# Mingqj/OcRFDet

Hardware: AMD Instinct MI355X
Metric: BEV voxels/sec + rendered views/sec, 6-cam 256x704 (higher is better)
Workload: dtype f32

## Files before the change

include/ocrf_hip.h:

```cpp
#ifndef OCRF_HIP_H
#define OCRF_HIP_H

#include <stddef.h>
#include <stdint.h>

#ifdef __cplusplus
extern "C" {
#endif

typedef void *ocrf_stream_t;

const char *ocrf_version(void);


void bev_pool_v2(int c, int n_intervals, const float *depth, const float *feat,
                 const int *ranks_depth, const int *ranks_feat, const int *ranks_bev,
                 const int *interval_starts, const int *interval_lengths, float *out);

void bev_pool_v2_grad(int c, int n_intervals, const float *out_grad, const float *depth,
                      const float *feat, const int *ranks_depth, const int *ranks_feat,
                      const int *ranks_bev, const int *interval_starts,
                      const int *interval_lengths, float *depth_grad, float *feat_grad);

int ocrf_bev_pool_v2(int c, int n_intervals, int n_points, long n_voxels, const float *depth, const float *feat,
// ... 166 lines not shown
                             float *heatmap, float *anno_box, long long *ind, unsigned char *mask, float *counts,
                             void *workspace, size_t workspace_bytes, ocrf_stream_t stream);
size_t ocrf_center_head_heatmap_loss_workspace_bytes(int B, int T, const int *ncls, int HW);
int ocrf_center_head_heatmap_loss(int B, int T, const int *ncls, int HW, const float *const *logits,
                                  const float *heatmap, const float *counts, float loss_weight, float *const *clipped,
                                  float *out, float *dens, void *workspace, size_t workspace_bytes,
                                  ocrf_stream_t stream);
int ocrf_center_head_heatmap_loss_backward(int B, int T, const int *ncls, int HW, const float *const *logits,
                                           const float *heatmap, const float *dens, const float *grad_out,
                                           float loss_weight, float *const *grad_logits, ocrf_stream_t stream);
size_t ocrf_center_head_reg_loss_workspace_bytes(int B, int T);
int ocrf_center_head_reg_loss(int B, int T, int HW, int max_objs, int with_velocity, const float *const *heads,
                              const float *anno_box, const long long *ind, const unsigned char *mask,
                              const float *code_weights, const float *counts, float loss_weight, float *out,
                              float *dens, void *workspace, size_t workspace_bytes, ocrf_stream_t stream);
int ocrf_center_head_reg_loss_backward(int B, int T, int HW, int max_objs, int with_velocity,
                                       const float *const *heads, const float *anno_box, const long long *ind,
                                       const unsigned char *mask, const float *code_weights, const float *dens,
                                       const float *grad_out, float loss_weight, float *const *grad_heads,
                                       ocrf_stream_t stream);

#define OCRF_CD_MAX_TASKS 8
#define OCRF_CD_MAX_CLASSES 8
#define OCRF_CD_MAX_NUM 1024
size_t ocrf_center_decode_workspace_bytes(int B, int T, int max_num, int post_max_size);
int ocrf_center_decode(int B, int T, const int *ncls, int H, int W, const float *const *heads, int with_velocity,
                       int norm_bbox, int max_num, int pre_max_size, int post_max_size, float out_size_factor,
                       const float *voxel_size, const float *pc_range, int has_coder_score_threshold,
                       float coder_score_threshold, const float *post_center_range, int has_score_threshold,
                       float score_threshold, const float *post_center_limit_range, const int *nms_circle,
                       const double *nms_threshold, const float *rescale_factor, float *boxes, float *scores,
                       int *labels, int *counts, void *workspace, size_t workspace_bytes, ocrf_stream_t stream);

int ocrf_lss_prepare(int B, int N, int D, int H, int W, const float *frustum, const float *cams,
                     const float *grid_lower_host, const float *grid_interval_host, int gx, int gy, int gz,
                     int *ranks_bev, int *ranks_depth, int *ranks_feat, int *interval_starts,
                     int *interval_lengths, int *counts, void *workspace, size_t workspace_bytes,
                     ocrf_stream_t stream);
size_t ocrf_lss_prepare_workspace_bytes(int B, int N, int D, int H, int W, int gx, int gy, int gz);
int ocrf_ht_prepare(int B, int N, int Z, int n_pillars, int Wf, int Hf, int D, const float *ref_points,
                    const float *cams, const float *pc_range_host, float w_in, float h_in, float depth0,
                    float depth1, int *ranks_bev, int *ranks_depth, int *ranks_feat, int *interval_starts,
                    int *interval_lengths, int *counts, void *workspace, size_t workspace_bytes,
                    ocrf_stream_t stream);
size_t ocrf_ht_prepare_workspace_bytes(int B, int n_pillars);

int ocrf_geometry_blocks(int B, int N, const float *rots, const float *trans, const float *intrins,
                         const float *post_rots, const float *post_trans, const float *bda, const float *c2w,
                         int H_in, int W_in, float znear, float zfar, float *lss_block, float *ht_block,
                         float *camera_rows, ocrf_stream_t stream);

int ocrf_hoa_channel_stats(const float *x, int B, int C, int Y, int X, float *stats,
                           ocrf_stream_t stream);
int ocrf_hoa_opacity_mask_gate(const float *x, const float *stats, const float *opacity_bev,
                               const float *conv_w, int k, int B, int C, int Y, int X, float *mask,
                               float *gated, ocrf_stream_t stream);

int ocrf_hoa_dw3x3(const float *x, const float *w, const float *bias, int B, int C, int Y, int X, float *y,
                   ocrf_stream_t stream);
int ocrf_hoa_dw3x3_wgrad_bands(int Y);
int ocrf_hoa_dw3x3_wgrad(const float *x, const float *dy, int B, int C, int Y, int X, float *partial,
                         ocrf_stream_t stream);

int ocrf_hoa_height_attention(const float *x, int B, int C, int hid, int Y, int X, const float *w1,
                              const float *w2, float *gate, float *gated, void *workspace,
                              size_t workspace_bytes, ocrf_stream_t stream);
size_t ocrf_hoa_height_attention_workspace_bytes(int B, int C);

int ocrf_hoa_unet_block(const float *src0, const float *gate0, int C0, int H0, int W0, int mode,
                        const float *up_w, const float *up_b, int Cup, const float *src1,
                        const float *gate1, int C1, const float *dw_w, const float *dw_b,
                        const float *pw_w, const float *pw_b, int Cout, const float *addend, float *out,
                        float *partial_max, int B, int H, int W, ocrf_stream_t stream);
int ocrf_hoa_unet_tiles(int H, int W);
int ocrf_hoa_v2b_weights_len(void);
size_t ocrf_hoa_v2b_workspace_bytes(int B, int H, int W);
int ocrf_hoa_v2b_forward(const float *x, const float *position, const float *weights, int B, int H, int W,
                         void *workspace, size_t workspace_bytes, float *out, ocrf_stream_t stream);
int ocrf_hoa_height_gate_from_tiles(int B, int C, int hid, int n_tiles, const float *partial_max,
                                    const float *w1, const float *w2, float *gate, ocrf_stream_t stream);
int ocrf_hoa_gated_conv1x1(const float *x, const float *gate, int B, int C, int H, int W, const float *w,
                           const float *bias, float *out, ocrf_stream_t stream);

int ocrf_hoa1_forward(const float *opacity, const float *alpha, const float *weights, int B, int Y, int X,
                      float offset_scale, float *att_workspace, float *out, ocrf_stream_t stream);
int ocrf_hoa1_weights_len(void);

int ocrf_ht_project(int B, int N, int Z, int n_pillars, const float *ref_points, const float *cams,
                    const float *pc_range, float w_in, float h_in, float depth0, float depth1,
                    float *pix, unsigned char *mask, float *voxel, ocrf_stream_t stream);


int ocrf_prefilter(const float *x, int BN, int D, int C, int HW, float depth_threshold,
                   float semantic_threshold, float *depth, float *filter_depth, float *semantic,
                   float *feat_channels_last, ocrf_stream_t stream);

int ocrf_pillar_sample_mean(const float *imgs, const float *pix, const unsigned char *mask, float *avg,
                            int B, int N, int C, int Hi, int Wi, int ZQ, ocrf_stream_t stream);

int ocrf_retain_valid_pixels(const float *imgs, const float *pix, const unsigned char *mask,
                             const int *cam_sel, float *out, int B, int N, int C, int H, int W, int ZQ,
                             ocrf_stream_t stream);

int ocrf_gauss_heads(const float *bev, const float *rgb_avg, const float *params, int B, int C, int Zh,
                     int YX, float *opacity, float *scales, float *rotations, float *color,
                     ocrf_stream_t stream);
// ... 146 lines not shown
```

ocrfdet_amd/csrc/hoa.hip:

```cpp
#include <hip/hip_runtime.h>

#include <algorithm>

#include "hoa_gate.h"
#include "launch.h"
#include "ocrf_hip.h"

namespace {

constexpr int kBlock = 256;
int g_mg_groups = 0, g_mg_threads = kBlock, g_stats_threads = kBlock;

__device__ __forceinline__ float sigmoidf_(float v) { return 1.0f / (1.0f + __expf(-v)); }

__global__ __launch_bounds__(kBlock) void hoa_channel_stats_kernel(const float* __restrict__ x, int C,
                                                                   long plane, float* __restrict__ stats) {
  OCRF_MAIN_CHAIN_PRIO();
  const long pix = (long)blockIdx.x * blockDim.x + threadIdx.x;
  const int b = blockIdx.y;
  if (pix >= plane) return;
  const float* p = x + (long)b * C * plane + pix;
  float sum = 0.f, mx = -INFINITY;
  int c = 0;
  for (; c + 16 <= C; c += 16) {
    float v[16];
#pragma unroll
    for (int u = 0; u < 16; ++u) v[u] = p[(long)(c + u) * plane];
#pragma unroll
    for (int u = 0; u < 16; ++u) {
      sum += v[u];
      mx = fmaxf(mx, v[u]);
    }
  }
  for (; c < C; ++c) {
    const float v = p[(long)c * plane];
    sum += v;
    mx = fmaxf(mx, v);
  }
  stats[((long)b * 2 + 0) * plane + pix] = sum / (float)C;
  stats[((long)b * 2 + 1) * plane + pix] = mx;
}

struct MaskGateD1 {
  const float* d1; const float* pm; const float* out_w; const float* out_b; const float* g_w1; const float* g_w2;
  float* opacity_out; int tiles;
};
template <int VEC, int KT, bool FAST = false, bool D1 = false>
__global__ __launch_bounds__(kBlock) void hoa_mask_gate_kernel(
    const float* __restrict__ x, const float* __restrict__ stats, const float* __restrict__ opacity_bev,
    const float* __restrict__ conv_w, int k_rt, int C, int Y, int X, int groups, int n_rows,
    float* __restrict__ mask, float* __restrict__ gated, MaskGateD1 dd) {
  OCRF_MAIN_CHAIN_PRIO();
  const int k = KT ? KT : k_rt;
  const int nt = (int)blockDim.x;
  extern __shared__ __attribute__((aligned(16))) float s_dyn[];
  const int r = k / 2, tw = FAST ? X + 8 : ((VEC == 4) ? ((X + k - 1 + 3) & ~3) : (X + k - 1));
  constexpr int PL = FAST ? 1 : 0;
  float* s_w = s_dyn;
  float* s_s = s_dyn + ((VEC == 4) ? ((2 * k * k + 3) & ~3) : 2 * k * k);
  const long plane = (long)Y * X;
  const int b = blockIdx.z / groups, g = blockIdx.z % groups;
  const long p0 = (long)blockIdx.x * nt * VEC;
  const int row0 = (int)(p0 / X) - r;
  for (int i = threadIdx.x; i < 2 * k * k; i += nt) s_w[i] = conv_w[i];
  const long pix_e = p0 + (long)threadIdx.x * VEC;
  const int cpg_e = (C + groups - 1) / groups;
  const int c0_e = g * cpg_e, c1_e = min(C, c0_e + cpg_e);
  float4 first[5];
  const bool pre = (VEC == 4) && gated && pix_e < plane && c0_e + 5 <= c1_e;
  if constexpr (VEC == 4) {
    if (pre) {
      const float* pe = x + (long)b * C * plane + pix_e;
#pragma unroll
      for (int u = 0; u < 5; ++u) first[u] = *reinterpret_cast<const float4*>(pe + (long)(c0_e + u) * plane);
    }
  }
  __shared__ __attribute__((aligned(16))) float s_red[16 * 4];
  __shared__ float s_g[4], s_ow[16];
  float4 d1v[D1 ? 4 : 1];
  float4 pmv[hoa_gate::kPmRounds];
  float owv = 0.f;
  if constexpr (D1) {
    const long pc = pix_e < plane ? pix_e : plane - VEC;
#pragma unroll
    for (int c = 0; c < 4; ++c) d1v[c] = *reinterpret_cast<const float4*>(dd.d1 + ((long)b * 4 + c) * plane + pc);
    hoa_gate::pm_issue<4>(dd.pm, b, dd.tiles, (int)threadIdx.x, pmv);
    const int t = (int)threadIdx.x & 15;
    const float* src = t < 4 ? dd.out_w + t : (t == 4 ? dd.out_b : (t < 9 ? dd.g_w1 + (t - 5) : dd.g_w2 + (min(t, 12) - 9)));
    owv = *src;
  }
  if constexpr (FAST) {
    const int n_items = 2 * n_rows * 64, x4 = X >> 2;
    float4* s_s4 = reinterpret_cast<float4*>(s_s);
// ... 260 lines not shown
        const int sx = xx + j - 1;
        if (sx < 0 || sx >= X) continue;
        acc[i * 3 + j] = fmaf(g, px[(long)sy * X + sx], acc[i * 3 + j]);
      }
    }
  }
#pragma unroll
  for (int t = 0; t < 10; ++t) {
    float v = acc[t];
    for (int off = 32; off > 0; off >>= 1) v += __shfl_down(v, off);
    if ((threadIdx.x & 63) == 0) s_acc[threadIdx.x >> 6][t] = v;
  }
  __syncthreads();
  if (threadIdx.x < 10) {
    float v = 0.f;
    for (int wv = 0; wv < kBlock / 64; ++wv) v += s_acc[wv][threadIdx.x];
    partial[((long)bc * gridDim.x + band) * 10 + threadIdx.x] = v;
  }
}

}

namespace ocrf {
void hoa_tune(int key, int value) {
  if (key == 20 && value >= 0) g_mg_groups = value;
  if (key == 21 && (value == 64 || value == 128 || value == 256)) g_mg_threads = value;
  if (key == 22 && (value == 64 || value == 128 || value == 256)) g_stats_threads = value;
}
}

extern "C" {

int ocrf_hoa_dw3x3(const float* x, const float* w, const float* bias, int B, int C, int Y, int X, float* y,
                   ocrf_stream_t stream_) {
  if (!x || !w || !y || B <= 0 || C <= 0 || Y <= 0 || X <= 0 || (long)B * C > 65535) return (int)hipErrorInvalidValue;
  ocrf::launch(OCRF_K_HOA_DW3X3, hoa_dw3x3_kernel, dim3((X + 63) / 64, (Y + 3) / 4, B * C), dim3(kBlock), 0,
               static_cast<hipStream_t>(stream_), x, w, bias, C, Y, X, y);
  return (int)hipGetLastError();
}

int ocrf_hoa_dw3x3_wgrad_bands(int Y) { return (Y + kDwBand - 1) / kDwBand; }

int ocrf_hoa_dw3x3_wgrad(const float* x, const float* dy, int B, int C, int Y, int X, float* partial,
                         ocrf_stream_t stream_) {
  if (!x || !dy || !partial || B <= 0 || C <= 0 || Y <= 0 || X <= 0 || (long)B * C > 65535)
    return (int)hipErrorInvalidValue;
  ocrf::launch(OCRF_K_HOA_DW3X3_WGRAD, hoa_dw3x3_wgrad_kernel, dim3(ocrf_hoa_dw3x3_wgrad_bands(Y), B * C),
               dim3(kBlock), 0, static_cast<hipStream_t>(stream_), x, dy, Y, X, partial);
  return (int)hipGetLastError();
}

int ocrf_hoa_channel_stats(const float* x, int B, int C, int Y, int X, float* stats, ocrf_stream_t stream_) {
  hipStream_t stream = static_cast<hipStream_t>(stream_);
  if (!x || !stats || B <= 0 || C <= 0 || Y <= 0 || X <= 0) return (int)hipErrorInvalidValue;
  const long plane = (long)Y * X;
  const int nt = g_stats_threads;
  ocrf::launch(OCRF_K_HOA_STATS, hoa_channel_stats_kernel, dim3((unsigned)((plane + nt - 1) / nt), B), dim3(nt), 0, stream,
               x, C, plane, stats);
  return (int)hipGetLastError();
}

int ocrf_hoa_opacity_mask_gate(const float* x, const float* stats, const float* opacity_bev,
                               const float* conv_w, int k, int B, int C, int Y, int X, float* mask,
                               float* gated, ocrf_stream_t stream_) {
  hipStream_t stream = static_cast<hipStream_t>(stream_);
  if (!x || !stats || !opacity_bev || !conv_w || !mask || k <= 0 || (k & 1) == 0 || k > 15 || B <= 0 ||
      C <= 0 || Y <= 0 || X <= 0)
    return (int)hipErrorInvalidValue;
  const long plane = (long)Y * X;
  const bool vec4 = (X % 4 == 0) && ((reinterpret_cast<uintptr_t>(x) | reinterpret_cast<uintptr_t>(gated)) & 15u) == 0 &&
                    (X + 6) * 14 * 2 * 4 <= 60 * 1024;
  const int threads = g_mg_threads;
  const int per_wg = threads * (vec4 ? 4 : 1);
  const int n_rows = (per_wg + X - 2) / X + 1 + (k - 1);
  const bool fast = vec4 && k == 7 && X <= 256 && (reinterpret_cast<uintptr_t>(stats) & 15u) == 0;
  const int tw = fast ? X + 8 : (vec4 ? ((X + k - 1 + 3) & ~3) : (X + k - 1));
  const size_t lds = (size_t)((vec4 ? ((2 * k * k + 3) & ~3) : 2 * k * k) + 2 * n_rows * tw) * sizeof(float);
  if (lds > 64 * 1024) return (int)hipErrorInvalidValue;
  int groups = gated ? ((C >= 40) ? 4 : (C >= 16 ? 2 : 1)) : 1;
  if (gated && g_mg_groups > 0) groups = std::min(g_mg_groups, C);
  const dim3 grid((unsigned)((plane + per_wg - 1) / per_wg), 1, (unsigned)(B * groups));
#define OCRF_MASK_GATE(V, K, F)                                                                                       \
  ocrf::launch(OCRF_K_HOA_MASK_GATE, hoa_mask_gate_kernel<V, K, F, false>, grid, dim3(threads), lds, stream, x, stats, opacity_bev, \
               conv_w, k, C, Y, X, groups, n_rows, mask, gated, MaskGateD1{})
  if (fast) OCRF_MASK_GATE(4, 7, true);
  else if (vec4 && k == 7) OCRF_MASK_GATE(4, 7, false);
  else if (vec4) OCRF_MASK_GATE(4, 0, false);
  else if (k == 7) OCRF_MASK_GATE(1, 7, false);
  else OCRF_MASK_GATE(1, 0, false);
#undef OCRF_MASK_GATE
  return (int)hipGetLastError();
}


size_t ocrf_hoa_height_attention_workspace_bytes(int B, int C) {
  return (size_t)B * C * 64 * sizeof(float);
}

int ocrf_hoa_height_attention(const float* x, int B, int C, int hid, int Y, int X, const float* w1,
                              const float* w2, float* gate, float* gated, void* workspace,
                              size_t workspace_bytes, ocrf_stream_t stream_) {
  hipStream_t stream = static_cast<hipStream_t>(stream_);
  if (!x || !w1 || !w2 || !gate || B <= 0 || C <= 0 || (C % 4) != 0 || C > 64 || hid <= 0 || 4 * hid > 64 ||
      Y <= 0 || X <= 0 || !workspace || workspace_bytes < ocrf_hoa_height_attention_workspace_bytes(B, C))
    return (int)hipErrorInvalidValue;
  const long plane = (long)Y * X;
  int n_split = (int)((plane + 4095) / 4096);
  if (n_split > 64) n_split = 64;
  float* partial = static_cast<float*>(workspace);
  ocrf::launch(OCRF_K_HOA_HEIGHT_MAX, hoa_height_max_kernel, dim3(n_split, B * C), dim3(kBlock), 0, stream, x,
               plane, n_split, partial);
// ... 774 lines not shown
```

ocrfdet_amd/csrc/step.hip:

```cpp
#include <hip/hip_runtime.h>

#include <cstdint>
#include <cstring>
#include <tuple>
#include <type_traits>
#include <utility>
#include <vector>

#include "ocrf_hip.h"

namespace {

constexpr int kMaxArgs = 40;
constexpr int kMaxStreams = 8;

template <typename T>
T word_as(uint64_t w) {
  if constexpr (std::is_pointer_v<T>) {
    return reinterpret_cast<T>(static_cast<uintptr_t>(w));
  } else if constexpr (std::is_same_v<T, float>) {
    const uint32_t b = static_cast<uint32_t>(w);
    float f;
    std::memcpy(&f, &b, 4);
    return f;
  } else {
    static_assert(std::is_integral_v<T>, "a step argument is a pointer, a float or an integer");
    return static_cast<T>(static_cast<int64_t>(w));
  }
}

template <typename F>
struct Signature;
template <typename R, typename... A>
struct Signature<R (*)(A...)> {
  static constexpr int n_args = int(sizeof...(A)) - 1;
  static_assert(std::is_same_v<R, int>, "an entry point a step holds returns its hipError_t as int");
  static_assert(std::is_same_v<std::tuple_element_t<sizeof...(A), std::tuple<void, A...>>, ocrf_stream_t>,
                "an entry point a step holds takes its ocrf_stream_t last");
  static_assert(n_args <= kMaxArgs, "raise kMaxArgs");

  template <R (*fn)(A...), size_t... I>
  static int call(const uint64_t* a, ocrf_stream_t s, std::index_sequence<I...>) {
    return fn(word_as<std::tuple_element_t<I, std::tuple<A...>>>(a[I])..., s);
  }
};

template <auto fn>
int invoke(const uint64_t* a, ocrf_stream_t s) {
  using Sig = Signature<decltype(fn)>;
  return Sig::template call<fn>(a, s, std::make_index_sequence<Sig::n_args>{});
}

struct FnInfo {
  const char* name;
  int n_args;
  int (*invoke)(const uint64_t* args, ocrf_stream_t stream);
};

#define OCRF_STEP_FN(fn) FnInfo{#fn, Signature<decltype(&fn)>::n_args, &invoke<&fn>}

const FnInfo kFns[] = {
    OCRF_STEP_FN(ocrf_bev_pool_v2_nchw_planned), OCRF_STEP_FN(ocrf_bev_pool_v2_nchw_mfma),
    OCRF_STEP_FN(ocrf_bev_pool_cell_weights),    OCRF_STEP_FN(ocrf_bev_pool_v2_nchw_panel),
    OCRF_STEP_FN(ocrf_rasterize_planned),        OCRF_STEP_FN(ocrf_hoa1_forward),
    OCRF_STEP_FN(ocrf_hoa_v2b_forward),          OCRF_STEP_FN(ocrf_hoa_channel_stats),
    OCRF_STEP_FN(ocrf_hoa_opacity_mask_gate),    OCRF_STEP_FN(ocrf_stream_write_value32),
    OCRF_STEP_FN(ocrf_raster_plan_build),        OCRF_STEP_FN(ocrf_rasterize_forward),
    OCRF_STEP_FN(ocrf_bev_pool_v2_nchw_dyn),     OCRF_STEP_FN(ocrf_lss_prepare),
    OCRF_STEP_FN(ocrf_ht_prepare),               OCRF_STEP_FN(ocrf_geometry_blocks),
    OCRF_STEP_FN(ocrf_rasterize_forward_sets),
};
#undef OCRF_STEP_FN
constexpr int kFnCount = int(sizeof(kFns) / sizeof(kFns[0]));

struct Cmd {
  int kind;
  int fn, slot, from, to;
  uint64_t a[kMaxArgs];
};

}

struct ocrf_step {
  std::vector<Cmd> cmds;
  hipEvent_t events[2 * kMaxStreams * kMaxStreams];
  int device;
};

extern "C" {

int ocrf_step_fn_id(const char* name) {
  if (!name) return -1;
  for (int i = 0; i < kFnCount; ++i)
    if (std::strcmp(name, kFns[i].name) == 0) return i;
  return -1;
}
int ocrf_step_fn_args(int fn) { return (fn >= 0 && fn < kFnCount) ? kFns[fn].n_args : -1; }

int ocrf_step_create(ocrf_step** out) {
  if (!out) return (int)hipErrorInvalidValue;
  ocrf_step* s = new ocrf_step();
  for (auto& e : s->events) e = nullptr;
  s->device = -1;
  *out = s;
  return 0;
}

void ocrf_step_destroy(ocrf_step* s) {
  if (!s) return;
  for (auto& e : s->events)
    if (e) (void)hipEventDestroy(e);
  delete s;
}

int ocrf_step_add_call(ocrf_step* s, int fn, int slot, int n_args, const uint64_t* args) {
  if (!s || fn < 0 || fn >= kFnCount || slot < 0 || slot >= kMaxStreams || n_args != kFns[fn].n_args || !args)
    return (int)hipErrorInvalidValue;
  Cmd c;
  std::memset(&c, 0, sizeof(c));
  c.kind = 0; c.fn = fn; c.slot = slot;
  std::memcpy(c.a, args, sizeof(uint64_t) * (size_t)n_args);
  s->cmds.push_back(c);
  return 0;
// ... 45 lines not shown
```

ocrfdet_amd/hoa.py:

```python
import torch
import torch.nn.functional as F
from torch import nn

from . import _lib
from .neck_ops import tall_linear

__all__ = ['HeightAttention', 'OpacityVoxelToBEVConverter', 'ObatinOpacityMask', 'DeformableAttention2D',
           'CPB', 'hoa1', 'spatial_gate']


def _f32c(t):
    return t.contiguous().float()


class _LaunchCache(dict):

    def __deepcopy__(self, memo):
        return _LaunchCache()

    def __reduce__(self):
        return (_LaunchCache, ())


class HeightAttention(nn.Module):
# ... 203 lines not shown
            keep.extend((out, pmax, gate))
            c0 = src0.shape[1] if src0 is not None else self.encoder1[0].in_channels
            h0, w0 = (src0.shape[2], src0.shape[3]) if src0 is not None else (H, W)
            args = [_lib.ptr(src0), _lib.ptr(gate0), c0, h0, w0, mode, _lib.ptr(up_w), _lib.ptr(up_b), cup,
                    _lib.ptr(src1), _lib.ptr(gate1), src1.shape[1] if src1 is not None else 0, _lib.ptr(dw_w),
                    _lib.ptr(dw_b), _lib.ptr(pw_w), _lib.ptr(pw_b), cout, _lib.ptr(None), _lib.ptr(out), _lib.ptr(pmax),
                    B, h, w]
            calls.append(('block', args, addend_slot))
            calls.append(('gate', [B, cout, ca.hid, n_tiles, _lib.ptr(pmax), _lib.ptr(w1), _lib.ptr(w2), _lib.ptr(gate)]))
            return out, gate
        with torch.no_grad():
            e1, g1 = block(None, None, 0, None, None, None, self.encoder1, self.ca1, 4, H, W, addend_slot=True)
            e2, g2 = block(e1, g1, 1, None, None, None, self.encoder2, self.ca2, 8, H // 2, W // 2)
            bt, gb = block(e2, g2, 1, None, None, None, self.bottleneck, self.ca_bottleneck, 16, H // 4, W // 4)
            d2, gd2 = block(bt, gb, 2, self.upconv2, e2, g2, self.decoder2, self.ca_dec2, 8, H // 2, W // 2)
            d1, gd1 = block(d2, gd2, 2, self.upconv1, e1, g1, self.decoder1, self.ca_dec1, 4, H, W)
            ow, ob = dev_f32(self.output_conv.weight.reshape(-1)), dev_f32(self.output_conv.bias)
        plan = dict(key=key, keep=keep, calls=calls,
                    out_args=[_lib.ptr(d1), _lib.ptr(gd1), B, 4, H, W, _lib.ptr(ow), _lib.ptr(ob)])
        cache['plan'] = plan
        return plan

    def _packed_v2b(self):
        cache = self.__dict__.get('_plan_cache')
        if cache is None:
            cache = self.__dict__['_plan_cache'] = _LaunchCache()
        tensors = cache.get('tensors')
        if tensors is None:
            tensors = cache['tensors'] = list(self.parameters()) + list(self.buffers())
        key = (tuple(t._version for t in tensors), tuple(t.data_ptr() for t in tensors))
        hit = cache.get('packed')
        if hit is not None and hit[0] == key:
            return hit[1]
        parts = []
        with torch.no_grad():
            for blk, ca in ((self.encoder1, self.ca1), (self.encoder2, self.ca2), (self.bottleneck, self.ca_bottleneck),
                            (self.decoder2, self.ca_dec2), (self.decoder1, self.ca_dec1)):
                parts.extend(t.reshape(-1) for t in self._folded(blk))
                parts.extend(t.reshape(-1) for t in ca._packed())
            for up in (self.upconv2, self.upconv1):
                parts.extend((up.weight.detach().float().reshape(-1), up.bias.detach().float().reshape(-1)))
            parts.extend((self.output_conv.weight.detach().float().reshape(-1), self.output_conv.bias.detach().float().reshape(-1)))
            packed = torch.cat([t.float() for t in parts])
            n = _lib.lib().ocrf_hoa_v2b_weights_len()
            assert 0 <= n - packed.numel() < 4, (n, packed.numel())
            packed = torch.cat((packed, packed.new_zeros(n - packed.numel()))).contiguous()
        cache['packed'] = (key, packed)
        return packed

    def _is_reference_architecture(self):
        e1 = self.encoder1[0]
        return (e1.in_channels == 13 and self.ca1.hid == self.ca1.q_in == 1 and self.ca_bottleneck.hid == 4)

    def _forward_fused(self, x, position):
        _lib.require_cuda(x, position)
        x, position = _f32c(x), _f32c(position)
        B, _, H, W = x.shape
        dev = x.device
        if self._is_reference_architecture() and H % 4 == 0 and W % 4 == 0:
            w = self._packed_v2b()
            out = torch.empty(B, 1, H, W, device=dev)
            ws = _lib.workspace.get(dev, _lib.lib().ocrf_hoa_v2b_workspace_bytes(B, H, W), 'hoa_v2b')
            _lib.launch('ocrf_hoa_v2b_forward', dev, x, position, w, B, H, W, ws, ws.numel(), out)
            return out
        return self._forward_blocks(x, position)

    def _forward_blocks(self, x, position):
        B, _, H, W = x.shape
        dev = x.device
        plan = self._plan(B, H, W, dev)
        out = torch.empty(B, 1, H, W, device=dev)
        for call in plan['calls']:
            if call[0] == 'block':
                args = call[1]
                if call[2]:
                    args = list(args)
                    args[0], args[17] = _lib.ptr(x), _lib.ptr(position)
                _lib.launch('ocrf_hoa_unet_block', dev, *args)
            else:
                _lib.launch('ocrf_hoa_height_gate_from_tiles', dev, *call[1])
        _lib.launch('ocrf_hoa_gated_conv1x1', dev, *plan['out_args'], out)
        return out


def channel_stats(x):
    _lib.require_cuda(x)
    B, C, Y, X = x.shape
    x = _f32c(x)
    stats = torch.empty(B, 2, Y, X, device=x.device)
    _lib.launch('ocrf_hoa_channel_stats', x.device, x, B, C, Y, X, stats)
    return stats


def spatial_gate(weight, x, addend, want_gated, stats=None, in_place=False):
    _lib.require_cuda(x, addend)
    B, C, Y, X = x.shape
    if in_place and (x.dtype != torch.float32 or not x.is_contiguous()):
        raise _lib.OcrfHipError('in_place gating needs a contiguous fp32 tensor')
    x, ob = _f32c(x), _f32c(addend)
    w = _f32c(weight)
    k = w.shape[-1]
    if stats is not None and (tuple(stats.shape) != (B, 2, Y, X) or stats.dtype != torch.float32 or not stats.is_contiguous()):
        raise _lib.OcrfHipError('stats must be the contiguous fp32 (B,2,Y,X) result of channel_stats(x)')
    mask = torch.empty(B, 1, Y, X, device=x.device)
    gated = (x if in_place else torch.empty_like(x)) if want_gated else None
    if stats is None:
        stats = torch.empty(B, 2, Y, X, device=x.device)
        _lib.launch('ocrf_hoa_channel_stats', x.device, x, B, C, Y, X, stats)
    _lib.launch('ocrf_hoa_opacity_mask_gate', x.device, x, stats, ob, w, k, B, C, Y, X, mask, gated)
    return mask, gated


class ObatinOpacityMask(nn.Module):
    def __init__(self, kernel_size=7):
        super().__init__()
        self.conv = nn.Conv2d(2, 1, kernel_size, padding=kernel_size // 2, bias=False)
        self.sigmoid = nn.Sigmoid()

    def _run(self, x, opacity_bev, want_gated, stats=None, in_place=False):
        _lib.require_cuda(x, opacity_bev)
        if torch.is_grad_enabled() and (x.requires_grad or opacity_bev.requires_grad or self.conv.weight.requires_grad):
            stats = torch.cat((x.mean(1, keepdim=True), torch.max(x, dim=1, keepdim=True)[0]), 1)
            mask = self.sigmoid(self.conv(stats) + opacity_bev)
            return mask, (x * mask if want_gated else None)
        return spatial_gate(self.conv.weight, x, opacity_bev, want_gated, stats=stats, in_place=in_place)

    def forward(self, x, opacity_bev):
        return self._run(x, opacity_bev, False)[0]

    def gate(self, x, opacity_bev, stats=None, in_place=False):
        return self._run(x, opacity_bev, True, stats=stats, in_place=in_place)


def _grid_like(t, dim=0):
    h, w = t.shape[-2:]
    xs = torch.arange(w, device=t.device)
    ys = torch.arange(h, device=t.device)
    gx, gy = torch.meshgrid(xs, ys, indexing='xy')
    return torch.stack((gx, gy), dim=dim).type_as(t)


def _normalize_grid(grid, dim=1, out_dim=-1):
    h, w = grid.shape[-2:]
    g0, g1 = grid.unbind(dim=dim)
    return torch.stack((2.0 * g0 / max(h - 1, 1) - 1.0, 2.0 * g1 / max(w - 1, 1) - 1.0), dim=out_dim)


class _Scale(nn.Module):
    def __init__(self, scale):
        super().__init__()
        self.scale = scale

    def forward(self, x):
        return x * self.scale


class CPB(nn.Module):

    def __init__(self, dim, *, heads, offset_groups, depth):
        super().__init__()
        self.heads, self.offset_groups = heads, offset_groups
        self.mlp = nn.ModuleList([nn.Sequential(nn.Linear(2, dim), nn.ReLU())])
        for _ in range(depth - 1):
            self.mlp.append(nn.Sequential(nn.Linear(dim, dim), nn.ReLU()))
        self.mlp.append(nn.Linear(dim, heads // offset_groups))

    def forward(self, grid_q, grid_kv):
        gq = grid_q.reshape(1, -1, grid_q.shape[-1])
        gk = grid_kv.reshape(grid_kv.shape[0], -1, grid_kv.shape[-1])
        pos = gq[:, :, None, :] - gk[:, None, :, :]
        bias = torch.sign(pos) * torch.log(pos.abs() + 1)
        for layer in self.mlp:
# ... 97 lines not shown
```

ocrfdet_amd/hotpath.py:

```python
import contextlib
import math

import numpy as np
import torch

from . import _lib, bevpool, gaussian_renderer, hoa, index_prep, raster_plan, synthetic
from .diff_gaussian_rasterization import pack_cameras, rasterize_sets, rasterize_views


class PoolPlan:

    def __init__(self, ranks_bev, ranks_depth, ranks_feat, starts, lengths, bev_shape):
        self.ranks_bev, self.ranks_depth, self.ranks_feat = ranks_bev, ranks_depth, ranks_feat
        self.starts, self.lengths = starts, lengths
        self.bev_shape = tuple(int(v) for v in bev_shape)
        self.device_plan = None
        self.mfma_plan = None

    @property
    def n_points(self):
        return int(self.ranks_bev.numel())

    @property
    def n_intervals(self):
        return int(self.starts.numel())

    def algorithmic_bytes(self, depth_numel, feat_numel):
        out = 1
        for v in self.bev_shape:
            out *= v
        return 4 * (depth_numel + feat_numel + 3 * self.n_points + 2 * self.n_intervals + out)


_STREAMS = {}


def shared_stream(device, role):
    key = (torch.device(device).index or 0, role)
    if key not in _STREAMS:
        _STREAMS[key] = torch.cuda.Stream(device)
    return _STREAMS[key]


class HotPath:
    def __init__(self, cfg, device, cams=None, index_prep_mode='cached', overlap=True, device_geometry=False,
                 render_mode='planned', render_guard='host', frame_motion=True, frame_offset=0, plan_margin=1.25,
                 ht_pool_backend=None, fuse_frames='auto', render_streams=1, blend_workgroups='auto',
                 lss_pool_backend=None, lss_mfma_group=2, plan_rebuild='never', hoa_first=None, one_call=True,
                 gaussians='init', alternate=None):
        self.cfg, self.device = cfg, torch.device(device)
        assert render_mode in ('planned', 'per_call') and render_guard in ('host', 'device')
        assert plan_rebuild in ('never', 'per_step')
        self.plan_rebuild = plan_rebuild
        assert gaussians in synthetic.GAUSSIAN_SETS
        self.gaussians = gaussians
        self.plan_bins = (4, 2)
        self.alternate = (gaussians == 'objects') if alternate is None else bool(alternate)
        self.phase = 0
        self.render_mode, self.render_guard, self.plan_margin = render_mode, render_guard, float(plan_margin)
        self.frame_motion, self.frame_offset = bool(frame_motion), int(frame_offset)
        self.overlap = bool(overlap) and self.device.type == 'cuda'
        if lss_pool_backend is None:
            lss_pool_backend = 'panel'
        if ht_pool_backend is None:
            ht_pool_backend = 'panel'
        assert ht_pool_backend in ('mfma', 'tile', 'panel') and lss_pool_backend in ('mfma', 'tile', 'panel')
        self.lss_panel_unit_cost = 8.0
        self.ht_pool_backend = ht_pool_backend
        self.lss_pool_backend, self.lss_mfma_group = lss_pool_backend, int(lss_mfma_group)
        self.hoa_first = hoa_first
        self.one_call = bool(one_call) and self.device.type == 'cuda'
        self._compiled = _lib.StepCache(self.device, size=4, seen_size=16, check=self._flat_outputs)
        self.fuse_frames = fuse_frames
        self.render_streams = max(1, int(render_streams))
        self.blend_workgroups = blend_workgroups
        self._busy = torch.zeros(1, dtype=torch.int32, device=self.device) if self.device.type == 'cuda' else None
        self.cams = list(range(cfg.n_cams)) if cams is None else list(cams)
        self.batch = cfg.batch * cfg.n_frames
        assert index_prep_mode in ('cached', 'per_step')
        self.index_prep_mode = index_prep_mode
        self.device_geometry = bool(device_geometry)
        self._side = []
        self._prep_stream = self._prep_stream2 = None
        self._prepare()

    def _prepare(self):
        cfg, dev = self.cfg, self.device
        r = synthetic.rig(cfg.n_cams, cfg.input_size, self.batch, frame_motion=self.frame_motion,
                          frame_offset=self.frame_offset)
        sel = self.cams
        g = {k: torch.from_numpy(r[k][:, sel] if r[k].ndim >= 3 and k != 'bda' else r[k]).to(dev)
             for k in ('rots', 'trans', 'intrins', 'post_rots', 'post_trans', 'bda', 'c2w')}
        self.geom = g
        X, Y, Z = cfg.bev_xyz
        Hf, Wf = cfg.feat_hw
        C = cfg.channels
        self._calib_host = [torch.from_numpy(r[k][:, sel] if k != 'bda' else r[k]) for k in
                            ('rots', 'trans', 'intrins', 'post_rots', 'post_trans', 'bda')]
        frustum = index_prep.create_frustum(cfg.grid['depth'], cfg.input_size, cfg.downsample)
        self._frustum_dev = frustum.to(dev).contiguous()
        self._ref_template = index_prep.get_reference_points_3d(Y, X, bs=1, num_points_in_pillar=cfg.num_height,
                                                                device='cpu')[0].to(dev).contiguous()
        self._grid = index_prep.grid_infos(cfg.grid)
        self._lss_bufs, self._ht_bufs = index_prep._RankBuffers(), index_prep._RankBuffers()
        self.lss, self.ht = self.prepare_indices_hip(sync=True)
        self._calib_dev = [t.to(dev).float().contiguous() for t in self._calib_host]
        for plan in (self.lss, self.ht):
            for name in ('ranks_bev', 'ranks_depth', 'ranks_feat', 'starts', 'lengths'):
                setattr(plan, name, getattr(plan, name).clone())
        lidar2img, img_aug, _, _ = index_prep.get_projection(*self._calib_host)
        ht_block = index_prep.ht_camera_block(lidar2img, img_aug).to(dev)
        _, _, voxel = index_prep.ht_project_hip(self._ref_template, ht_block, self.batch, len(sel), list(cfg.pc_range),
                                                cfg.input_size, cfg.grid['depth'])
        self.voxel_xyz = voxel

        if cfg.render:
            self._prepare_render(r)
        if cfg.hoa:
            self._prepare_hoa()

    def _prepare_hoa(self, seed=0):
        cfg, dev = self.cfg, self.device
        X, Y, _ = cfg.bev_xyz
        torch.manual_seed(seed)
        self.hoa_mods = dict(
            dca=hoa.DeformableAttention2D(dim=cfg.num_height, dim_head=8, heads=1, dropout=0.1, downsample_factor=4,
                                          offset_scale=4, offset_groups=None, offset_kernel_size=6),
            v2b=hoa.OpacityVoxelToBEVConverter(input_channel=cfg.num_height), mask=hoa.ObatinOpacityMask())
        for m in self.hoa_mods.values():
            m.to(dev).eval()
        g = torch.Generator(device='cpu').manual_seed(seed)
        self.alpha_lidar = torch.rand(self.batch, cfg.num_height, Y, X, generator=g).to(dev)
        self._opac_flat = None
        self.bev_pos1 = (torch.randn(self.batch, 4, Y, X, generator=g) * 0.1).to(dev)

    @torch.no_grad()
    def hoa_opacity_bev(self):
        cfg = self.cfg
        X, Y, _ = cfg.bev_xyz
        m = self.hoa_mods
        if self._opac_flat is None:
            self._opac_flats = [torch.stack([fg['opacity'].view(cfg.num_height, Y, X) for fg in fgs]).reshape(-1, 1).contiguous()
                                for fgs in self.frame_gauss_sets]
            self._opac_flat = self._opac_flats[self.phase]
        oa = hoa.hoa1(m['dca'], self._opac_flat, self.alpha_lidar, cfg.num_height, Y, X)
        return m['v2b'](oa, self.bev_pos1)

    @torch.no_grad()
    def hoa_step(self, geom_feat, opacity_bev=None):
        if opacity_bev is None:
            opacity_bev = self.hoa_opacity_bev()
        _, gated = self.hoa_mods['mask'].gate(geom_feat, opacity_bev)
        return gated, opacity_bev

    def _prepare_render(self, r, convention='corrected', seed=0):
        cfg, dev = self.cfg, self.device
        H, W = cfg.input_size
        self.frame_cams = []
        n_sets = 2 if self.alternate else 1
        self.frame_gauss_sets = [[] for _ in range(n_sets)]
        P = self.voxel_xyz.shape[1] * self.voxel_xyz.shape[2]
        t = lambda a: torch.from_numpy(a).to(dev)
        for b in range(self.batch):
            vms, pms, tfx, tfy = [], [], [], []
            for n in self.cams:
                K = r['intrins'][b, n].astype(np.float64)
                c2w = r['c2w'][b, n].astype(np.float64)
                if convention == 'corrected':
                    s, crop = r['resize'], r['crop_h']
                    K = np.array([[K[0, 0] * s, 0, K[0, 2] * s], [0, K[1, 1] * s, K[1, 2] * s - crop], [0, 0, 1.0]])
                    w2c = np.linalg.inv(c2w)
                    c2w_arg = np.eye(4)
                    c2w_arg[:3, :3] = c2w[:3, :3]
                    c2w_arg[:3, 3] = w2c[:3, 3]
                else:
                    c2w_arg = c2w
                cam = gaussian_renderer.camera_from_calibration(K.astype(np.float32), c2w_arg.astype(np.float32), H, W)
                vms.append(cam['world_view_transform']), pms.append(cam['full_proj_transform'])
                tfx.append(math.tan(float(cam['FovX']) * 0.5)), tfy.append(math.tan(float(cam['FovY']) * 0.5))
            rc = dict(vm=torch.stack(vms).to(dev), pm=torch.stack(pms).to(dev), tfx=tfx, tfy=tfy)
            rc['packed'] = pack_cameras(rc['vm'], rc['pm'], tfx, tfy, H, W, dev)
            self.frame_cams.append(rc)
            xyz_np = self.voxel_xyz[b].reshape(-1, 3).cpu().numpy()
            for ph in range(n_sets):
                gs = synthetic.grid_gaussians(self.gaussians, xyz_np,
                                              seed + (self.frame_offset + b if self.frame_motion else 0) + 1000 * ph)
                self.frame_gauss_sets[ph].append({k: t(v) for k, v in gs.items()})
        self.frame_gauss = self.frame_gauss_sets[0]
        self.render_cams, self.gauss = self.frame_cams[0], self.frame_gauss[0]
        self.bg = torch.zeros(3, device=dev)
        self.render_convention = convention
        self.render_plans = None
        self._opac_flat = None

    def _plans(self):
        if self.render_plans is None:
            H, W = self.cfg.input_size
            n_cam = len(self.cams)
            same = all(torch.equal(self.voxel_xyz[b], self.voxel_xyz[0]) for b in range(1, self.batch))
            fuse = True if self.fuse_frames == 'auto' else bool(self.fuse_frames)
            per = max(1, 32 // n_cam) if (same and fuse) else 1
            self.render_plans = []
            for f0 in range(0, self.batch, per):
                fr = list(range(f0, min(f0 + per, self.batch)))
                cams = torch.cat([self.frame_cams[b]['packed'] for b in fr])
                alts = [{k: torch.stack([fgs[b][k] for b in fr]).contiguous() for k in ('rgb', 'opacity', 'scales', 'rotations')}
# ... 189 lines not shown
                                                  cfg.grid['depth'], Wf, Hf, cfg.D, buffers=self._ht_bufs, sync=False)

    def prepare_indices_hip(self, sync=True):
        cfg, dev = self.cfg, self.device
        X, Y, Z = cfg.bev_xyz
        Hf, Wf = cfg.feat_hw
        args = self._calib_host
        B, N = args[1].shape[:2]
        lss_block, ht_block = self._camera_blocks()
        lss = self._prepare_lss(lss_block)
        ht = self._prepare_ht(ht_block)
        if not sync:
            return lss, ht
        counts = torch.stack((lss[1], ht[1])).cpu()
        return (PoolPlan(*self._or_empty(index_prep._trim(lss[0], counts[0])), (self.batch, Z, Y, X, cfg.channels)),
                PoolPlan(*self._or_empty(index_prep._trim(ht[0], counts[1])), (self.batch, 1, Y, X, cfg.channels)))

    def pool_step(self, depth, feat, prepared=None):
        if self.index_prep_mode == 'per_step':
            (lv, lc), (hv, hc) = prepared if prepared is not None else self.prepare_indices_hip(sync=False)
            lss = bevpool.bev_pool_v2_device_counts(depth, feat, lv[1], lv[2], lv[0], self.lss.bev_shape, lv[3], lv[4], lc)
            ht = bevpool.bev_pool_v2_device_counts(depth, feat, hv[1], hv[2], hv[0], self.ht.bev_shape, hv[3], hv[4], hc)
            return lss, ht
        C = self.lss.bev_shape[-1]
        if (self.lss_pool_backend == 'panel' and self.ht_pool_backend == 'panel' and C in (64, 80, 96, 128)
                and self.lss.n_points and self.ht.n_points):
            bevpool.bev_pool_cell_weights(depth, self._panel_plan(self.lss), self._panel_plan(self.ht))
            return self.pool(self.lss, depth, feat, weights_ready=True), self.pool(self.ht, depth, feat, weights_ready=True)
        return self.pool(self.lss, depth, feat), self.pool(self.ht, depth, feat)

    def step(self, depth, feat):
        if self.cfg.render and self.render_mode == 'planned':
            self._plans()
        if not self.one_call:
            return self._step_eager(depth, feat)
        if (self._compiled.refused is None and self.index_prep_mode == 'per_step'
                and not (self.device_geometry and hasattr(self, '_calib_dev'))):
            self._compiled.refused = 'per-step calibration algebra on the host is issued call by call'
        out = self._compiled(self._step_key(depth, feat), self._step_streams(torch.cuda.current_stream(self.device)),
                             lambda rec: self._step_eager(depth, feat, rec))
        for entry in (self.render_plans or []) if self.cfg.render and self.render_mode == 'planned' else []:
            entry[0]._host_guarded = entry[0]._host_guarded or self.render_guard == 'host'
        return out

    @property
    def one_call_refused(self):
        return self._compiled.refused

    def _step_key(self, depth, feat):
        bw = self.blend_workgroups
        return (depth.data_ptr(), feat.data_ptr(), tuple(depth.shape), tuple(feat.shape), depth.dtype, feat.dtype, self.phase,
                self.index_prep_mode, self.plan_rebuild, self.overlap, bw if isinstance(bw, (int, str)) else tuple(bw),
                self.render_mode, self.render_guard, self.hoa_first, self.lss_pool_backend, self.ht_pool_backend,
                self.render_streams, self.fuse_frames, self.device_geometry)

    def _forks(self):
        return self.overlap and self.cfg.render

    def _prep_forks(self):
        return (self.index_prep_mode == 'per_step' and self.cfg.hoa and self.overlap and self.device_geometry
                and hasattr(self, '_calib_dev'))

    def _step_streams(self, cur):
        st = [cur]
        if self._forks():
            if not self._side:
                self._side = [shared_stream(self.device, 'render' if k == 0 else f'render{k}')
                              for k in range(self.render_streams)]
            st += list(self._side)
        if self._prep_forks():
            if self._prep_stream is None:
                self._prep_stream = shared_stream(self.device, 'prep')
                self._prep_stream2 = shared_stream(self.device, 'prep2')
            st += [self._prep_stream, self._prep_stream2]
        return st

    @staticmethod
    def _flat_outputs(out):
        for o in out:
            if torch.is_tensor(o):
                yield o
            elif isinstance(o, dict):
                yield from (v for k, v in o.items() if torch.is_tensor(v) and k != 'status')
            elif isinstance(o, (list, tuple)):
                yield from HotPath._flat_outputs(o)

    def _step_eager(self, depth, feat, rec=None):
        fork = self._forks()
        self._rec = rec
        if not fork:
            main = self._main_chain(depth, feat)
            rendered = [self.render()] if self.cfg.render else []
            return tuple(main[:2]) + tuple(rendered) + tuple(main[2:])
        cur = torch.cuda.current_stream(self.device)
        self._set_busy(1)
        if not self._side:
            self._side = [shared_stream(self.device, 'render' if k == 0 else f'render{k}')
                          for k in range(self.render_streams)]
        if getattr(self, '_fork_ev', None) is None:
            self._fork_ev = torch.cuda.Event()
            self._join_ev = [torch.cuda.Event() for _ in self._side]
        self._fork_ev.record(cur)
        for k, side in enumerate(self._side):
            side.wait_event(self._fork_ev)
            if rec is not None:
                rec.fork(0, 1 + k)
        rendered = self.render([self._side[b % len(self._side)] for b in range(self.batch)])
        main = self._main_chain(depth, feat)
        self._set_busy(0)
        for k, (side, ev) in enumerate(zip(self._side, self._join_ev)):
            ev.record(side)
            cur.wait_event(ev)
            if rec is not None:
                rec.join(1 + k, 0)
        for frame in rendered:
            for v in frame.values():
                if torch.is_tensor(v):
                    v.record_stream(cur)
        return tuple(main[:2]) + (rendered,) + tuple(main[2:])

    def _main_chain(self, depth, feat):
        prepared = None
        if self._prep_forks():
            cur0 = torch.cuda.current_stream(self.device)
            self._step_streams(cur0)
            p1, p2 = self._prep_stream, self._prep_stream2
            rec = getattr(self, '_rec', None)
            s1 = 1 + (len(self._side) if self._forks() else 0)
            p1.wait_stream(cur0)
            p2.wait_stream(cur0)
            if rec is not None:
                rec.fork(0, s1)
                rec.fork(0, s1 + 1)
            with torch.cuda.stream(p1):
                lss_block, ht_block = self._camera_blocks()
                blocks_ready = torch.cuda.Event()
                blocks_ready.record(p1)
                ht_block.record_stream(p2)
                if rec is not None:
                    rec.fork(s1, s1 + 1)
                lv, lc = self._prepare_lss(lss_block)
                lss = bevpool.bev_pool_v2_device_counts(depth, feat, lv[1], lv[2], lv[0], self.lss.bev_shape, lv[3], lv[4], lc)
            p2.wait_event(blocks_ready)
            with torch.cuda.stream(p2):
                hv, hc = self._prepare_ht(ht_block)
                ht = bevpool.bev_pool_v2_device_counts(depth, feat, hv[1], hv[2], hv[0], self.ht.bev_shape, hv[3], hv[4], hc,
                                                       scratch_tag='bev_pool_nchw_b')
            prepared = True
        hoa_first = self.hoa_first
        if hoa_first is None:
            hoa_first = self.render_mode != 'planned' or self.index_prep_mode == 'per_step'
        ob = self.hoa_opacity_bev() if (self.cfg.hoa and hoa_first) else None
        if prepared is not None:
            main = torch.cuda.current_stream(self.device)
            rec = getattr(self, '_rec', None)
            s1 = 1 + (len(self._side) if self._forks() else 0)
            main.wait_stream(self._prep_stream)
            if rec is not None:
                rec.join(s1, 0)
            main.wait_stream(self._prep_stream2)
            if rec is not None:
                rec.join(s1 + 1, 0)
            lss.record_stream(main)
            ht.record_stream(main)
        else:
            lss, ht = self.pool_step(depth, feat, prepared)
        if self.cfg.hoa and not hoa_first:
            ob = self.hoa_opacity_bev()
        out = [lss, ht]
        if self.cfg.hoa:
            out.extend(self.hoa_step(ht, ob))
        return out

    @property
    def bev_voxels_per_step(self):
        X, Y, Z = self.cfg.bev_xyz
        return self.batch * Z * Y * X


class ShardedHotPath:

    def __init__(self, cfg, device, rank, world, index_prep_mode='cached', render_mode='planned', render_guard='host',
                 sparse_exchange=True, collectives=None, one_call=True):
        from . import sharding
        self.cfg, self.device, self.rank, self.world = cfg, torch.device(device), rank, world
        self._one_call = bool(one_call) and self.device.type == 'cuda' and index_prep_mode == 'cached'
        self._segments = _lib.StepCache(self.device, size=16, seen_size=32)
        X, Y, Z = cfg.bev_xyz
        C = cfg.channels
        self.n_frames = cfg.batch * cfg.n_frames
        self.planes_lss = Z * C
        self.planes_pool = (Z + 1) * C
        self.opacity_plane = self.planes_pool if cfg.hoa else None
        self.plan = sharding.CameraFramePlan(cfg.n_cams, self.n_frames, world, self.planes_pool + (1 if cfg.hoa else 0))
        self.exchange = sharding.BevExchange(self.plan, rank, self.device, (Y, X), collectives=collectives)
        one = synthetic.PathConfig(**{**cfg.__dict__, 'batch': 1, 'n_frames': 1, 'hoa': False})
        self.subs = {f: HotPath(one, self.device, cams=self.plan.cams_of(rank, f), index_prep_mode=index_prep_mode,
                                overlap=False, frame_offset=f, render_mode=render_mode, render_guard=render_guard,
                                one_call=False)
                     for f in self.plan.frames_of(rank)}
        self.my_frames = self.plan.frames_of(rank)
        self.base = None
        if cfg.hoa:
            self.base = HotPath(synthetic.PathConfig(**{**cfg.__dict__, 'render': cfg.render or cfg.hoa}), self.device,
                                cams=[0], index_prep_mode='cached', overlap=False, one_call=False)
            fr = self.my_frames
            Zh = cfg.num_height
            self._hoa_in = None
            if fr:
                opac = torch.stack([self.base.frame_gauss[f]['opacity'].view(Zh, Y, X) for f in fr]).reshape(-1, 1).contiguous()
                self._hoa_in = (opac, self.base.alpha_lidar[fr].contiguous(), self.base.bev_pos1[fr].contiguous())
        self.hoa_launch_frames = 0
        self._side = shared_stream(self.device, 'render') if self.device.type == 'cuda' and cfg.render else None
        self._busy = None
        if self._side is not None and render_mode == 'planned':
            self._busy = torch.zeros(1, dtype=torch.int32, device=self.device)
            for sub in self.subs.values():
                sub._yield_word = self._busy
        self.sparse_exchange = bool(sparse_exchange) and self.plan.any_shared and index_prep_mode == 'cached'
        if self.sparse_exchange:
            ex, touched = self.exchange, {}
# ... 235 lines not shown
```

Measured before the change: 388.2 million.

## Defer HOA v2b output conv into channel-stats kernel

Skips writing the v2b converter's final opacity output and instead computes it (gated 4-channel conv with bias) inside the channel-stats kernel, which already walks every BEV pixel. This removes a separate output pass and its launch from the HOA chain. The stats loop is also reworked into larger unrolled channel rounds (80/64/32/16) with a clamped tail, which raises register pressure. A deferred-opacity object is threaded through the Python hot path, and it is forward-only.

Measured after the change: 391.6 million (median of 6 runs). Within noise of the previous version (+0.9%).

```diff
diff --git a/include/ocrf_hip.h b/include/ocrf_hip.h
--- a/include/ocrf_hip.h
+++ b/include/ocrf_hip.h
@@ -242,6 +242,9 @@
 
 int ocrf_hoa_channel_stats(const float *x, int B, int C, int Y, int X, float *stats,
                            ocrf_stream_t stream);
+int ocrf_hoa_channel_stats_v2b(const float *x, int B, int C, int Y, int X, float *stats, const void *workspace,
+                               size_t workspace_bytes, const float *weights, float *opacity_out,
+                               ocrf_stream_t stream);
 int ocrf_hoa_opacity_mask_gate(const float *x, const float *stats, const float *opacity_bev,
                                const float *conv_w, int k, int B, int C, int Y, int X, float *mask,
                                float *gated, ocrf_stream_t stream);
diff --git a/ocrfdet_amd/csrc/hoa.hip b/ocrfdet_amd/csrc/hoa.hip
--- a/ocrfdet_amd/csrc/hoa.hip
+++ b/ocrfdet_amd/csrc/hoa.hip
@@ -13,32 +13,79 @@
 
 __device__ __forceinline__ float sigmoidf_(float v) { return 1.0f / (1.0f + __expf(-v)); }
 
-__global__ __launch_bounds__(kBlock) void hoa_channel_stats_kernel(const float* __restrict__ x, int C,
-                                                                   long plane, float* __restrict__ stats) {
+struct StatsD1 {
+  const float* d1; const float* pm; const float* out_w; const float* out_b; const float* g_w1; const float* g_w2;
+  float* opacity_out; int tiles;
+};
+template <int N>
+__device__ __forceinline__ void stats_round(const float* __restrict__ pc, long plane, unsigned pix, float& sum, float& mx) {
+  float v[N];
+#pragma unroll
+  for (int u = 0; u < N; ++u) v[u] = (pc + (long)u * plane)[pix];
+#pragma unroll
+  for (int u = 0; u < N; ++u) {
+    sum += v[u];
+    mx = fmaxf(mx, v[u]);
+  }
+}
+template <bool D1>
+__global__ __launch_bounds__(kBlock) void hoa_channel_stats_kernel(const float* __restrict__ x, int C, long plane,
+                                                                   float* __restrict__ stats, StatsD1 dd) {
   OCRF_MAIN_CHAIN_PRIO();
-  const long pix = (long)blockIdx.x * blockDim.x + threadIdx.x;
-  const int b = blockIdx.y;
-  if (pix >= plane) return;
-  const float* p = x + (long)b * C * plane + pix;
+  const int t = (int)threadIdx.x, b = blockIdx.y;
+  const long pix = (long)blockIdx.x * blockDim.x + t;
+  const unsigned pc = (unsigned)(pix < plane ? pix : plane - 1);
+  __shared__ __attribute__((aligned(16))) float s_red[16 * 4];
+  __shared__ float s_g[4], s_ow[16];
+  float d1v[4] = {0.f, 0.f, 0.f, 0.f};
+  float4 pmv[hoa_gate::kPmRounds];
+  float owv = 0.f;
+  if constexpr (D1) {
+#pragma unroll
+    for (int c = 0; c < 4; ++c) d1v[c] = (dd.d1 + ((long)b * 4 + c) * plane)[pc];
+    hoa_gate::pm_issue<4>(dd.pm, b, dd.tiles, t, pmv);
+    const int k = t & 15;
+    const float* src = k < 4 ? dd.out_w + k : (k == 4 ? dd.out_b : (k < 9 ? dd.g_w1 + (k - 5) : dd.g_w2 + (min(k, 12) - 9)));
+    owv = *src;
+  }
+  const float* p = x + (long)b * C * plane;
   float sum = 0.f, mx = -INFINITY;
   int c = 0;
-  for (; c + 16 <= C; c += 16) {
-    float v[16];
-#pragma unroll
-    for (int u = 0; u < 16; ++u) v[u] = p[(long)(c + u) * plane];
-#pragma unroll
-    for (int u = 0; u < 16; ++u) {
-      sum += v[u];
-      mx = fmaxf(mx, v[u]);
-    }
-  }
-  for (; c < C; ++c) {
-    const float v = p[(long)c * plane];
-    sum += v;
-    mx = fmaxf(mx, v);
-  }
-  stats[((long)b * 2 + 0) * plane + pix] = sum / (float)C;
-  stats[((long)b * 2 + 1) * plane + pix] = mx;
+  for (; c + 80 <= C; c += 80) stats_round<80>(p + (long)c * plane, plane, pc, sum, mx);
+  if (c + 64 <= C) { stats_round<64>(p + (long)c * plane, plane, pc, sum, mx); c += 64; }
+  if (c + 32 <= C) { stats_round<32>(p + (long)c * plane, plane, pc, sum, mx); c += 32; }
+  if (c + 16 <= C) { stats_round<16>(p + (long)c * plane, plane, pc, sum, mx); c += 16; }
+  if (c < C) {
+    float v[15];
+#pragma unroll
+    for (int u = 0; u < 15; ++u) v[u] = (p + (long)min(c + u, C - 1) * plane)[pc];
+#pragma unroll
+    for (int u = 0; u < 15; ++u) {
+      if (c + u < C) {
+        sum += v[u];
+        mx = fmaxf(mx, v[u]);
+      }
+    }
+  }
+  if (pix < plane) {
+    stats[((long)b * 2 + 0) * plane + pix] = sum / (float)C;
+    stats[((long)b * 2 + 1) * plane + pix] = mx;
+  }
+  if constexpr (D1) {
+    if (t < 16) s_ow[t] = owv;
+    hoa_gate::pm_reduce_rows<4>(dd.pm, b, dd.tiles, t, pmv, s_red);
+    __syncthreads();
+    if (t < 64) {
+      const float gt = hoa_gate::gate_of_lane<4>(s_red, s_ow + 5, s_ow + 9, t);
+      if (t < 4) s_g[t] = gt;
+    }
+    __syncthreads();
+    float acc = s_ow[4];
+#pragma unroll
+    for (int k = 0; k < 4; ++k) acc = fmaf(d1v[k] * s_g[k], s_ow[k], acc);
+    asm volatile("" : "+v"(acc));
+    if (pix < plane) dd.opacity_out[(long)b * plane + pix] = acc;
+  }
 }
 
 struct MaskGateD1 {
@@ -405,11 +452,27 @@
 
 int ocrf_hoa_channel_stats(const float* x, int B, int C, int Y, int X, float* stats, ocrf_stream_t stream_) {
   hipStream_t stream = static_cast<hipStream_t>(stream_);
-  if (!x || !stats || B <= 0 || C <= 0 || Y <= 0 || X <= 0) return (int)hipErrorInvalidValue;
+  if (!x || !stats || B <= 0 || C <= 0 || Y <= 0 || X <= 0 || (long)Y * X >= (1l << 30)) return (int)hipErrorInvalidValue;
   const long plane = (long)Y * X;
   const int nt = g_stats_threads;
-  ocrf::launch(OCRF_K_HOA_STATS, hoa_channel_stats_kernel, dim3((unsigned)((plane + nt - 1) / nt), B), dim3(nt), 0, stream,
-               x, C, plane, stats);
+  ocrf::launch(OCRF_K_HOA_STATS, hoa_channel_stats_kernel<false>, dim3((unsigned)((plane + nt - 1) / nt), B), dim3(nt), 0,
+               stream, x, C, plane, stats, StatsD1{});
+  return (int)hipGetLastError();
+}
+
+int ocrf_hoa_channel_stats_v2b(const float* x, int B, int C, int Y, int X, float* stats, const void* workspace,
+                               size_t workspace_bytes, const float* weights, float* opacity_out, ocrf_stream_t stream_) {
+  hipStream_t stream = static_cast<hipStream_t>(stream_);
+  if (!x || !stats || !workspace || !weights || !opacity_out || B <= 0 || B > 65535 || C <= 0 || Y < 4 || X < 4 || (Y % 4) ||
+      (X % 4) || (long)Y * X >= (1l << 30) || workspace_bytes < ocrf_hoa_v2b_workspace_bytes(B, Y, X) ||
+      (reinterpret_cast<uintptr_t>(workspace) & 15u))
+    return (int)hipErrorInvalidValue;
+  const long plane = (long)Y * X;
+  StatsD1 dd;
+  ocrf::v2b_deferred_pointers(workspace, weights, B, Y, X, &dd.d1, &dd.pm, &dd.tiles, &dd.out_w, &dd.out_b, &dd.g_w1, &dd.g_w2);
+  dd.opacity_out = opacity_out;
+  ocrf::launch(OCRF_K_HOA_STATS, hoa_channel_stats_kernel<true>, dim3((unsigned)((plane + kBlock - 1) / kBlock), B),
+               dim3(kBlock), 0, stream, x, C, plane, stats, dd);
   return (int)hipGetLastError();
 }
 
diff --git a/ocrfdet_amd/csrc/step.hip b/ocrfdet_amd/csrc/step.hip
--- a/ocrfdet_amd/csrc/step.hip
+++ b/ocrfdet_amd/csrc/step.hip
@@ -68,7 +68,7 @@
     OCRF_STEP_FN(ocrf_raster_plan_build),        OCRF_STEP_FN(ocrf_rasterize_forward),
     OCRF_STEP_FN(ocrf_bev_pool_v2_nchw_dyn),     OCRF_STEP_FN(ocrf_lss_prepare),
     OCRF_STEP_FN(ocrf_ht_prepare),               OCRF_STEP_FN(ocrf_geometry_blocks),
-    OCRF_STEP_FN(ocrf_rasterize_forward_sets),
+    OCRF_STEP_FN(ocrf_rasterize_forward_sets),   OCRF_STEP_FN(ocrf_hoa_channel_stats_v2b),
 };
 #undef OCRF_STEP_FN
 constexpr int kFnCount = int(sizeof(kFns) / sizeof(kFns[0]));
diff --git a/ocrfdet_amd/hoa.py b/ocrfdet_amd/hoa.py
--- a/ocrfdet_amd/hoa.py
+++ b/ocrfdet_amd/hoa.py
@@ -279,18 +279,27 @@
         e1 = self.encoder1[0]
         return (e1.in_channels == 13 and self.ca1.hid == self.ca1.q_in == 1 and self.ca_bottleneck.hid == 4)
 
-    def _forward_fused(self, x, position):
+    def _forward_fused(self, x, position, deferred=False):
         _lib.require_cuda(x, position)
         x, position = _f32c(x), _f32c(position)
         B, _, H, W = x.shape
         dev = x.device
         if self._is_reference_architecture() and H % 4 == 0 and W % 4 == 0:
             w = self._packed_v2b()
+            ws = _lib.workspace.get(dev, _lib.lib().ocrf_hoa_v2b_workspace_bytes(B, H, W), 'hoa_v2b')
+            if deferred:
+                _lib.launch('ocrf_hoa_v2b_forward', dev, x, position, w, B, H, W, ws, ws.numel(), None)
+                return DeferredOpacityBEV(ws, w, (B, 1, H, W))
             out = torch.empty(B, 1, H, W, device=dev)
-            ws = _lib.workspace.get(dev, _lib.lib().ocrf_hoa_v2b_workspace_bytes(B, H, W), 'hoa_v2b')
             _lib.launch('ocrf_hoa_v2b_forward', dev, x, position, w, B, H, W, ws, ws.numel(), out)
             return out
         return self._forward_blocks(x, position)
+
+    def forward_deferred(self, x, position):
+        if not self.training and x.is_cuda and not (torch.is_grad_enabled() and (
+                x.requires_grad or any(p.requires_grad for p in self.parameters()))):
+            return self._forward_fused(x, position, deferred=True)
+        return self.forward(x, position)
 
     def _forward_blocks(self, x, position):
         B, _, H, W = x.shape
@@ -310,12 +319,27 @@
         return out
 
 
-def channel_stats(x):
+class DeferredOpacityBEV:
+    __slots__ = ('workspace', 'weights', 'shape', 'out')
+
+    def __init__(self, workspace, weights, shape):
+        self.workspace, self.weights, self.shape, self.out = workspace, weights, tuple(shape), None
+
+
+def channel_stats(x, opacity=None):
     _lib.require_cuda(x)
     B, C, Y, X = x.shape
     x = _f32c(x)
     stats = torch.empty(B, 2, Y, X, device=x.device)
-    _lib.launch('ocrf_hoa_channel_stats', x.device, x, B, C, Y, X, stats)
+    if opacity is None:
+        _lib.launch('ocrf_hoa_channel_stats', x.device, x, B, C, Y, X, stats)
+        return stats
+    if opacity.shape != (B, 1, Y, X) or opacity.workspace.device != x.device:
+        raise _lib.OcrfHipError(f'deferred opacity BEV {opacity.shape} does not belong to x {tuple(x.shape)}')
+    if opacity.out is None:
+        opacity.out = torch.empty(opacity.shape, device=x.device)
+    ws = opacity.workspace
+    _lib.launch('ocrf_hoa_channel_stats_v2b', x.device, x, B, C, Y, X, stats, ws, ws.numel(), opacity.weights, opacity.out)
     return stats
 
 
@@ -345,6 +369,13 @@
         self.sigmoid = nn.Sigmoid()
 
     def _run(self, x, opacity_bev, want_gated, stats=None, in_place=False):
+        if isinstance(opacity_bev, DeferredOpacityBEV):
+            if torch.is_grad_enabled() and (x.requires_grad or self.conv.weight.requires_grad):
+                raise _lib.OcrfHipError('a deferred opacity BEV is forward-only: use the converter\'s forward under autograd')
+            if opacity_bev.out is None or stats is None:
+                own = channel_stats(x, opacity=opacity_bev)
+                stats = own if stats is None else stats
+            return spatial_gate(self.conv.weight, x, opacity_bev.out, want_gated, stats=stats, in_place=in_place)
         _lib.require_cuda(x, opacity_bev)
         if torch.is_grad_enabled() and (x.requires_grad or opacity_bev.requires_grad or self.conv.weight.requires_grad):
             stats = torch.cat((x.mean(1, keepdim=True), torch.max(x, dim=1, keepdim=True)[0]), 1)
diff --git a/ocrfdet_amd/hotpath.py b/ocrfdet_amd/hotpath.py
--- a/ocrfdet_amd/hotpath.py
+++ b/ocrfdet_amd/hotpath.py
@@ -69,6 +69,7 @@
         self.ht_pool_backend = ht_pool_backend
         self.lss_pool_backend, self.lss_mfma_group = lss_pool_backend, int(lss_mfma_group)
         self.hoa_first = hoa_first
+        self.hoa_out_conv = 'stats'
         self.one_call = bool(one_call) and self.device.type == 'cuda'
         self._compiled = _lib.StepCache(self.device, size=4, seen_size=16, check=self._flat_outputs)
         self.fuse_frames = fuse_frames
@@ -135,7 +136,8 @@
         self.bev_pos1 = (torch.randn(self.batch, 4, Y, X, generator=g) * 0.1).to(dev)
 
     @torch.no_grad()
-    def hoa_opacity_bev(self):
+    def hoa_opacity_bev(self, deferred=False):
+        assert self.hoa_out_conv in ('stats', 'own')
         cfg = self.cfg
         X, Y, _ = cfg.bev_xyz
         m = self.hoa_mods
@@ -144,14 +146,16 @@
                                 for fgs in self.frame_gauss_sets]
             self._opac_flat = self._opac_flats[self.phase]
         oa = hoa.hoa1(m['dca'], self._opac_flat, self.alpha_lidar, cfg.num_height, Y, X)
+        if deferred and self.hoa_out_conv == 'stats':
+            return m['v2b'].forward_deferred(oa, self.bev_pos1)
         return m['v2b'](oa, self.bev_pos1)
 
     @torch.no_grad()
     def hoa_step(self, geom_feat, opacity_bev=None):
         if opacity_bev is None:
-            opacity_bev = self.hoa_opacity_bev()
+            opacity_bev = self.hoa_opacity_bev(deferred=True)
         _, gated = self.hoa_mods['mask'].gate(geom_feat, opacity_bev)
-        return gated, opacity_bev
+        return gated, (opacity_bev.out if isinstance(opacity_bev, hoa.DeferredOpacityBEV) else opacity_bev)
 
     def _prepare_render(self, r, convention='corrected', seed=0):
         cfg, dev = self.cfg, self.device
@@ -447,7 +451,7 @@
         return (depth.data_ptr(), feat.data_ptr(), tuple(depth.shape), tuple(feat.shape), depth.dtype, feat.dtype, self.phase,
                 self.index_prep_mode, self.plan_rebuild, self.overlap, bw if isinstance(bw, (int, str)) else tuple(bw),
                 self.render_mode, self.render_guard, self.hoa_first, self.lss_pool_backend, self.ht_pool_backend,
-                self.render_streams, self.fuse_frames, self.device_geometry)
+                self.render_streams, self.fuse_frames, self.device_geometry, self.hoa_out_conv)
 
     def _forks(self):
         return self.overlap and self.cfg.render
@@ -545,7 +549,7 @@
         hoa_first = self.hoa_first
         if hoa_first is None:
             hoa_first = self.render_mode != 'planned' or self.index_prep_mode == 'per_step'
-        ob = self.hoa_opacity_bev() if (self.cfg.hoa and hoa_first) else None
+        ob = self.hoa_opacity_bev(deferred=True) if (self.cfg.hoa and hoa_first) else None
         if prepared is not None:
             main = torch.cuda.current_stream(self.device)
             rec = getattr(self, '_rec', None)
@@ -561,7 +565,7 @@
         else:
             lss, ht = self.pool_step(depth, feat, prepared)
         if self.cfg.hoa and not hoa_first:
-            ob = self.hoa_opacity_bev()
+            ob = self.hoa_opacity_bev(deferred=True)
         out = [lss, ht]
         if self.cfg.hoa:
             out.extend(self.hoa_step(ht, ob))
```
